# homenc/HElib

Hardware: NVIDIA H100
Metric: ctxt_mults_per_s (higher is better)
Workload: dtype u64

## Files before the change

### helib_b200/csrc/hb_device.cuh

```cuda
#pragma once

#ifdef HB_SIM
#include "cusim.h"
#define HB_SMEM_DECL
#define HB_SMEM ((u64*)cusim::smem_)
#define HB_NOINLINE __attribute__((noinline))
#define HB_GRID_CONSTANT
#else
#define HB_GRID_CONSTANT __grid_constant__
#define HB_NOINLINE __noinline__
#include <cuda_runtime.h>
#define HB_LAUNCH(kernel, grid, block, smem, stream, ...) kernel<<<(grid), (block), (smem), (stream)>>>(__VA_ARGS__)
#define HB_SMEM_DECL extern __shared__ unsigned long long hb_smem_[];
#define HB_SMEM hb_smem_
#endif

#include <stdint.h>

typedef unsigned long long u64;
typedef long long i64;

#define HB_MAXROWS 64
#ifndef HB_MAXB
#define HB_MAXB 64
// ... 262 lines not shown
  const size_t rowoff = (size_t)pi << J.logN;
  const u64* src = J.src[blockIdx.z] + rowoff;
  u64* dst = J.dst[blockIdx.z] + rowoff;
  const unsigned u0 = blockIdx.x << J.logwb;

  for (int e = tid; e < (wb << lb); e += nthr) {
    int v = e >> J.logwb, ub = e & (wb - 1);
    unsigned c = hb_brev(v, lb);
    T[ub * RS + c] = src[((size_t)v << n1) + u0 + ub];
  }
  __syncthreads();
  for (int s = lb - 1; s >= 0; s--) {
    const int logt = lb - 1 - s;
    for (int e = tid; e < (wb << (lb - 1)); e += nthr) {
      int ub = e >> (lb - 1), bf = e & ((BLK >> 1) - 1);
      int i = bf >> logt, o = bf & ((1 << logt) - 1);
      int j = (i << (logt + 1)) + o;
      unsigned b = hb_brev(u0 + ub, n1);
      ulonglong2 tw = P.iw[((size_t)1 << (n1 + s)) + ((size_t)b << s) + i];
      u64* pa = T + ub * RS + j;
      u64* pb = pa + (1 << logt);
      u64 U = *pa, V = *pb;
      *pa = hb_addmod(U, V, q);
      *pb = hb_mul_shoup(hb_submod(U, V, q), tw.x, tw.y, q);
    }
    __syncthreads();
  }
  for (int e = tid; e < (wb << lb); e += nthr) {
    int ub = e >> lb, c = e & (BLK - 1);
    unsigned b = hb_brev(u0 + ub, n1);
    dst[((size_t)b << lb) + c] = T[ub * RS + c];
  }
}

__device__ __forceinline__ void hb_cols_load(u64* T, const u64* src, int n1, int lb, int logw, unsigned c0) {
  const int cnt = 1 << (n1 + logw);
  for (int e = threadIdx.x; e < cnt; e += blockDim.x) {
    int i1 = e >> logw, c = e & ((1 << logw) - 1);
    T[e] = src[((size_t)i1 << lb) + c0 + c];
  }
}
__device__ __forceinline__ void hb_cols_store(const u64* T, u64* dst, int n1, int lb, int logw, unsigned c0) {
  const int cnt = 1 << (n1 + logw);
  for (int e = threadIdx.x; e < cnt; e += blockDim.x) {
    int i1 = e >> logw, c = e & ((1 << logw) - 1);
    dst[((size_t)i1 << lb) + c0 + c] = T[e];
  }
}

__global__ void __launch_bounds__(HB_THREADS) k_fwd_cols(const HbPrimeDev* __restrict__ primes, HbColsJob J) {
  HB_SMEM_DECL
  u64* T = HB_SMEM;
  const int n1 = J.logN - J.log_blk;
  const int pi = J.rows.prime[blockIdx.y];
  const HbPrimeDev P = primes[pi];
  const size_t rowoff = (size_t)pi << J.logN;
  const unsigned c0 = blockIdx.x << J.logw;
  hb_cols_load(T, J.src[blockIdx.z] + rowoff, n1, J.log_blk, J.logw, c0);
  __syncthreads();
  hb_tile_fwd_cols(T, n1, J.logw, P.fw, P.q);
  hb_cols_store(T, J.dst[blockIdx.z] + rowoff, n1, J.log_blk, J.logw, c0);
}

__global__ void __launch_bounds__(HB_THREADS) k_inv_cols(const HbPrimeDev* __restrict__ primes, HbColsJob J) {
  HB_SMEM_DECL
  u64* T = HB_SMEM;
  const int n1 = J.logN - J.log_blk;
  const int pi = J.rows.prime[blockIdx.y];
  const HbPrimeDev P = primes[pi];
  const size_t rowoff = (size_t)pi << J.logN;
  const unsigned c0 = blockIdx.x << J.logw;
  hb_cols_load(T, J.src[blockIdx.z] + rowoff, n1, J.log_blk, J.logw, c0);
  __syncthreads();
  hb_tile_inv_cols(T, n1, J.logw, P.iw, P.q);
  const int cnt = 1 << (n1 + J.logw);
  for (int e = threadIdx.x; e < cnt; e += blockDim.x) T[e] = hb_mul_shoup(T[e], P.ninv, P.ninv_s, P.q);
  __syncthreads();
  hb_cols_store(T, J.dst[blockIdx.z] + rowoff, n1, J.log_blk, J.logw, c0);
}


#define HB_MAXL 66

__device__ HB_NOINLINE int hb_crt_exact(const HbConvDev* cv, const u64* y, int ystride, int* sign, u64* xout, int Lout, int positive) {
  const int n = cv->n, L = cv->L;
  u64 X[HB_MAXL + 1];
  for (int l = 0; l <= L; l++) X[l] = 0;
  for (int j = 0; j < n; j++) {
    const u64 yj = y[(size_t)j * ystride];
    const u64* Qj = cv->Qj + (size_t)j * L;
    u64 carry = 0;
    for (int l = 0; l < L; l++) {
      u64 lo = yj * Qj[l], hi = __umul64hi(yj, Qj[l]);
      u64 s = X[l] + lo; u64 c1 = s < lo;
      u64 s2 = s + carry; u64 c2 = s2 < carry;
      X[l] = s2; carry = hi + c1 + c2;
    }
    X[L] += carry;
  }
  int v = 0;
  for (;;) {
    bool neg = (X[L] >> 63) != 0;
    int cmp = 0;
    if (neg) cmp = -1;
    else if (X[L] != 0) cmp = 1;
    else {
      for (int l = L - 1; l >= 0; l--) {
        u64 bl = positive ? cv->Q[l] : cv->Qhalf[l];
        if (X[l] != bl) { cmp = X[l] < bl ? -1 : 1; break; }
      }
      if (positive && cmp == 0) cmp = 1;
    }
    if (cmp <= 0) break;
    u64 borrow = 0;
    for (int l = 0; l < L; l++) {
      u64 a = X[l], b = cv->Q[l];
      u64 d = a - b; u64 b1 = a < b;
      u64 d2 = d - borrow; u64 b2 = d < borrow;
      X[l] = d2; borrow = b1 + b2;
    }
    X[L] -= borrow;
    v++;
  }
  bool neg = (X[L] >> 63) != 0;
  bool zero = true;
  for (int l = 0; l <= L; l++) if (X[l]) zero = false;
  *sign = neg ? -1 : (zero ? 0 : 1);
  if (xout) {
    u64 ext = neg ? ~0ULL : 0ULL;
    for (int l = 0; l < Lout; l++) xout[l] = l <= L ? X[l] : ext;
  }
  return v;
}

__device__ __forceinline__ i64 hb_conv_v(const HbConvDev* cv, const u64* y, int ystride, u64* stats, double* frac = nullptr, bool bgv = true) {
  const int n = cv->n;
  u64 shi = 0, slo = 0;
  for (int j = 0; j < n; j++) {
    const u64 yj = y[(size_t)j * ystride];
    u64 m = cv->fmul[j];
    int sh = cv->fshift[j];
    u64 lo = yj * m, hi = __umul64hi(yj, m);
    u64 f = sh == 0 ? lo : ((lo >> sh) | (hi << (64 - sh)));
    slo += f;
    shi += (slo < f) ? 1ULL : 0ULL;
  }
  u64 F = slo + 0x8000000000000000ULL;
  i64 v = (i64)(shi + (F < slo ? 1ULL : 0ULL));
  const u64 margin = 4ULL * (u64)n;
  int sign = 2;
  if (F >= 0 - margin) {
    const i64 ve = hb_crt_exact(cv, y, ystride, &sign, nullptr, 0, 0);
    if (ve != v) F = 0;
    v = ve;
    if (stats) atomicAdd(stats, 1ULL);
  }
  if (bgv && cv->has_p) {
    const u64 p = cv->p;
    u64 hi = 0, lo = 0;
    for (int j = 0; j < n; j++) hb_mac128(hi, lo, y[(size_t)j * ystride], cv->cp[j]);
    hb_mac128(hi, lo, (u64)v, cv->negQ_p);
    u64 u = hb_reduce128(hi, lo, p, cv->p_c64, cv->p_c64_s, cv->p_one_s);
    if (u != 0) {
      u = hb_mul_shoup(u, cv->Qinv_p, cv->Qinv_p_s, p);
      const u64 half = p >> 1;
      bool minus = u > half;
      if (!minus && (p & 1ULL) == 0 && u == half) {
        if (sign == 2) {
          if (F >= 0x8000000000000000ULL) sign = 1;
          else if (F < 0x8000000000000000ULL - margin) sign = -1;
          else { hb_crt_exact(cv, y, ystride, &sign, nullptr, 0, 0); if (stats) atomicAdd(stats, 1ULL); }
        }
        minus = sign < 0;
      }
      const i64 v2 = minus ? (i64)u - (i64)p : (i64)u;
      v += v2;
      if (frac) *frac = (double)(i64)(F ^ 0x8000000000000000ULL) * 5.421010862427522e-20 - (double)v2;
      return v;
    }
  }
  if (frac) *frac = (double)(i64)(F ^ 0x8000000000000000ULL) * 5.421010862427522e-20;
  return v;
}

__global__ void __launch_bounds__(HB_THREADS) k_conv(const HbPrimeDev* __restrict__ primes, HbConvJob J) {
  HB_SMEM_DECL
  const HbConvDev* cv = J.cv;
  const int n = cv->n, nt = cv->nt;
  const int n1 = J.logN - J.log_blk, lb = J.log_blk, logw = J.logw;
  const int TILE = 1 << (n1 + logw);
  u64* Y = HB_SMEM;
  i64* Vb = (i64*)(Y + (size_t)n * TILE);
  u64* W = (u64*)(Vb + TILE);
  const int tid = threadIdx.x, nthr = blockDim.x;
  const unsigned c0 = blockIdx.x << logw;
  const u64* src = J.src[blockIdx.y];
  u64* dst = J.dst[blockIdx.y];

  for (int j = 0; j < n; j++) {
    const int pi = cv->src_prime[j];
    const HbPrimeDev P = primes[pi];
    u64* T = Y + (size_t)j * TILE;
    hb_cols_load(T, src + ((size_t)pi << J.logN), n1, lb, logw, c0);
    __syncthreads();
    if (J.src_is_y) continue;
    hb_tile_inv_cols(T, n1, logw, P.iw, P.q);
    const u64 t = cv->tn[j], ts = cv->tn_s[j];
    for (int e = tid; e < TILE; e += nthr) T[e] = hb_mul_shoup(T[e], t, ts, P.q);
  }
  __syncthreads();
  double* fr = J.frac[blockIdx.y];
  for (int e = tid; e < TILE; e += nthr) {
    double f;
    Vb[e] = hb_conv_v(cv, Y + e, TILE, J.stats, fr ? &f : nullptr);
    if (fr) fr[((size_t)(e >> logw) << lb) + c0 + (e & ((1 << logw) - 1))] = f;
  }
  __syncthreads();
  for (int t = 0; t < nt; t++) {
    const int pi = cv->tgt_prime[t];
    const HbPrimeDev P = primes[pi];
    const u64* ct = cv->c + (size_t)t * n;
    const u64 nq = cv->negQ[t], pq = cv->Qmod[t];
    for (int e = tid; e < TILE; e += nthr) {
      u64 hi = 0, lo = 0;
      for (int j = 0; j < n; j++) hb_mac128(hi, lo, Y[(size_t)j * TILE + e], ct[j]);
      i64 v = Vb[e];
      if (v >= 0) hb_mac128(hi, lo, (u64)v, nq);
      else hb_mac128(hi, lo, (u64)(-v), pq);
      W[e] = hb_reduce128(hi, lo, P);
    }
    __syncthreads();
    hb_tile_fwd_cols(W, n1, logw, P.fw, P.q);
    hb_cols_store(W, dst + ((size_t)pi << J.logN), n1, lb, logw, c0);
    __syncthreads();
  }
}

struct HbCrtTabs { const u64* t; const u64* t_s; };
__global__ void __launch_bounds__(HB_THREADS) k_crt(const HbPrimeDev* __restrict__ primes, HbCrtJob J, HbCrtTabs tabs) {
  const HbConvDev* cv = J.cv;
  const int n = cv->n;
  size_t k = (size_t)blockIdx.x * blockDim.x + threadIdx.x;
  if (k >= (size_t)J.N) return;
  u64 y[HB_MAXROWS];
  for (int j = 0; j < n; j++) {
    int pi = cv->src_prime[j];
    u64 q = primes[pi].q;
    y[j] = hb_mul_shoup(J.src[(size_t)pi * J.N + k], tabs.t[j], tabs.t_s[j], q);
  }
  int sign;
  hb_crt_exact(cv, y, 1, &sign, J.out + k * J.Lout, J.Lout, J.positive);
}

__global__ void __launch_bounds__(HB_THREADS) k_crt_modp(const HbPrimeDev* __restrict__ primes, HbCrtJob J, HbCrtTabs tabs) {
// ... 548 lines not shown
```

### helib_b200/csrc/hb_device_v1.cuh

```cuda
#pragma once
#include <utility>
#include "hb_device.cuh"

#define HB1_RS 17
#define HB1_BS 273

__device__ __forceinline__ void hb_group_sync(int group, int nthreads) {
#ifdef HB_SIM
  cusim::bar_sync(1 + group, nthreads);
#else
  asm volatile("bar.sync %0, %1;" ::"r"(1 + group), "r"(nthreads) : "memory");
#endif
}

__device__ __forceinline__ void hb1_mac128(u64& hi, u64& lo, u64 a, u64 b) {
#ifdef HB_SIM
  hb_mac128(hi, lo, a, b);
#else
  asm("{\n\t.reg .u64 pl, ph;\n\t"
      "mul.lo.u64 pl, %2, %3;\n\t"
      "mul.hi.u64 ph, %2, %3;\n\t"
      "add.cc.u64 %0, %0, pl;\n\t"
      "addc.u64 %1, %1, ph;\n\t}"
      : "+l"(lo), "+l"(hi)
// ... 495 lines not shown
  u64* peer[8][HB_MAXB];
};

template <bool SP>
__global__ void __launch_bounds__(256, 2) k1_fwd_cols(const HbPrimeDev* __restrict__ primes, const HB_GRID_CONSTANT Hb1ColsJob J) {
  HB_SMEM_DECL
  u64* T = HB_SMEM;
  const int tid = threadIdx.x;
  const int pi = J.rows.prime[blockIdx.y];
  const HbPrimeDev P = primes[pi];
  HB1_MOD(M, P);
  const size_t rowoff = (size_t)pi << J.logN;
  const unsigned c0 = blockIdx.x << 4;
  const int c = tid & 15, x = tid >> 4;
  Hb1TwPtr tw1;
  tw1.p[0] = P.fw + 1; tw1.p[1] = P.fw + 2; tw1.p[2] = P.fw + 4; tw1.p[3] = P.fw + 8;
  Hb1TwReg tw2;
  tw2.load([&](int k, int g) { return P.fw[(16 << k) + (x << k) + g]; });
  for (int it = blockIdx.z; it < J.nitems; it += gridDim.z) {
    const u64* src = J.src[it] + rowoff + c0 + c;
    u64* dst = J.dst[it] + rowoff + c0 + c;
    u64 a[16];
    hb1_unroll<16>([&](auto r) { a[r] = src[(size_t)(16 * r + x) << 8]; });
    hb1_r16_fwd<SP>(a, tw1, M);
    hb1_unroll<16>([&](auto r) { T[c * HB1_BS + HB1_RS * r + x] = a[r]; });
    __syncthreads();
    hb1_unroll<16>([&](auto l) { a[l] = T[c * HB1_BS + HB1_RS * x + l]; });
    hb1_r16_fwd<SP>(a, tw2, M);
    hb1_unroll<16>([&](auto l) { dst[(size_t)(16 * x + l) << 8] = a[l]; });
    __syncthreads();
  }
}
template <bool SP>
__global__ void __launch_bounds__(256, 2) k1_inv_cols(const HbPrimeDev* __restrict__ primes, const HB_GRID_CONSTANT Hb1ColsJob J) {
  HB_SMEM_DECL
  u64* T = HB_SMEM;
  const int tid = threadIdx.x;
  const int pi = J.rows.prime[blockIdx.y];
  const HbPrimeDev P = primes[pi];
  const u64 q = P.q; HB1_MOD(M, P);
  const size_t rowoff = (size_t)pi << J.logN;
  const unsigned c0 = blockIdx.x << 4;
  const int c = tid & 15, x = tid >> 4;
  Hb1TwPtr tw1;
  tw1.p[0] = P.iw + 1; tw1.p[1] = P.iw + 2; tw1.p[2] = P.iw + 4; tw1.p[3] = P.iw + 8;
  Hb1TwReg tw2;
  tw2.load([&](int k, int g) { return P.iw[(16 << k) + (x << k) + g]; });
  for (int it = blockIdx.z; it < J.nitems; it += gridDim.z) {
    const u64* src = J.src[it] + rowoff + c0 + c;
    u64* dst = J.dst[it] + rowoff + c0 + c;
    u64 a[16];
    hb1_unroll<16>([&](auto l) { a[l] = src[(size_t)(16 * x + l) << 8]; });
    hb1_r16_inv<SP>(a, tw2, M);
    hb1_unroll<16>([&](auto l) { T[c * HB1_BS + HB1_RS * x + l] = a[l]; });
    __syncthreads();
    hb1_unroll<16>([&](auto r) { a[r] = T[c * HB1_BS + HB1_RS * r + x]; });
    hb1_r16_inv<SP>(a, tw1, M);
    const u64 fm = J.has_scal ? J.scal[blockIdx.y] : P.ninv, fs = J.has_scal ? J.scal_s[blockIdx.y] : P.ninv_s;
    hb1_unroll<16>([&](auto r) {
      const u64 v = hb_mul_shoup(a[r], fm, fs, q);
      const size_t o = (size_t)(16 * r + x) << 8;
      dst[o] = v;
      for (int p = 0; p < J.npeers; p++) J.peer[p][it][rowoff + c0 + c + o] = v;
    });
    __syncthreads();
  }
}

#define HB1C_BS 276
#define HB1_TS (4 * HB1C_BS)
#define HB1_VS 260

struct Hb1ConvJob {
  const HbConvDev* cv;
  int logN, ngroups;
  int nitems;
  const u64* src[HB_MAXB];
  u64* dst[HB_MAXB];
  u64* stats;
  int src_is_y;
  double* frac[HB_MAXB];
};

template <bool SP>
__global__ void __launch_bounds__(640, 1) k1_conv(const HbPrimeDev* __restrict__ primes, const HB_GRID_CONSTANT Hb1ConvJob J) {
  HB_SMEM_DECL
  const HbConvDev* cv = J.cv;
  const int n = cv->n, nt = cv->nt, NG = J.ngroups;
  u64* Y = HB_SMEM;
  i64* Vb = (i64*)(Y + (size_t)n * HB1_TS);
  u64* W = (u64*)(Vb + 4 * HB1_VS);
  const int tid = threadIdx.x;
  const int grp = tid >> 6, gt = tid & 63;
  const int c = gt & 3, x = gt >> 2;
  const unsigned c0 = blockIdx.x << 2;
  const u64* src = J.src[blockIdx.y];
  u64* dst = J.dst[blockIdx.y];

  for (int j = grp; j < n; j += NG) {
    const int pi = cv->src_prime[j];
    const HbPrimeDev P = primes[pi];
    const u64 q = P.q; HB1_MOD(M, P);
    const u64* s = src + ((size_t)pi << J.logN) + c0 + c;
    u64* Yj = Y + (size_t)j * HB1_TS + c * HB1C_BS;
    u64 a[16];
    hb1_unroll<16>([&](auto l) { a[l] = s[(size_t)(16 * x + l) << 8]; });
    if (J.src_is_y) {
      hb1_unroll<16>([&](auto l) { Yj[HB1_RS * x + l] = a[l]; });
      continue;
    }
    {
      Hb1TwPtr tw;
      tw.p[0] = P.iw + 16 + x; tw.p[1] = P.iw + 32 + 2 * x; tw.p[2] = P.iw + 64 + 4 * x; tw.p[3] = P.iw + 128 + 8 * x;
      hb1_r16_inv<SP>(a, tw, M);
    }
    hb1_unroll<16>([&](auto l) { Yj[HB1_RS * x + l] = a[l]; });
    hb_group_sync(grp, 64);
    hb1_unroll<16>([&](auto r) { a[r] = Yj[HB1_RS * r + x]; });
    {
      Hb1TwPtr tw;
      tw.p[0] = P.iw + 1; tw.p[1] = P.iw + 2; tw.p[2] = P.iw + 4; tw.p[3] = P.iw + 8;
      hb1_r16_inv<SP>(a, tw, M);
    }
    const u64 t = cv->tn[j], ts = cv->tn_s[j];
    hb1_unroll<16>([&](auto r) { Yj[HB1_RS * r + x] = hb_mul_shoup(a[r], t, ts, q); });
  }
  __syncthreads();
  for (int e = tid; e < 1024; e += blockDim.x) {
    const int cc = e >> 8, i1 = e & 255;
    double* fr = J.frac[blockIdx.y];
    double f;
    Vb[cc * HB1_VS + i1] = hb_conv_v(cv, Y + cc * HB1C_BS + HB1_RS * (i1 >> 4) + (i1 & 15), HB1_TS, J.stats, fr ? &f : nullptr);
    if (fr) fr[((size_t)i1 << 8) + c0 + cc] = f;
  }
  __syncthreads();
  u64* Wg = W + (size_t)grp * HB1_TS + c * HB1C_BS;
  for (int t = grp; t < nt; t += NG) {
    const int pi = cv->tgt_prime[t];
    const HbPrimeDev P = primes[pi];
    HB1_MOD(M, P);
    const u64* ct = cv->c + (size_t)t * n;
    u64 a[16];
    {
      const u64 negq = cv->negQ[t], posq = cv->Qmod[t];
      hb1_unroll<2>([&](auto h) {
        u64 ahi[8], alo[8];
        hb1_unroll<8>([&](auto r) {
          const i64 v = Vb[c * HB1_VS + 16 * (8 * h + r) + x];
          const u64 m = v >= 0 ? (u64)v : (u64)(-v);
          const u64 f = v >= 0 ? negq : posq;
          if ((m >> 32) == 0) {
            const u64 p0 = hb1_mulwide((unsigned)m, (unsigned)f);
            const u64 p1 = hb1_mulwide((unsigned)m, (unsigned)(f >> 32)) + (p0 >> 32);
            alo[r] = (p1 << 32) | (unsigned)p0; ahi[r] = p1 >> 32;
          } else { alo[r] = m * f; ahi[r] = __umul64hi(m, f); }
        });
        for (int j = 0; j < n; j++) {
          const u64 cj = ct[j];
          const u64* Yj = Y + (size_t)j * HB1_TS + c * HB1C_BS + x + HB1_RS * 8 * h;
          hb1_unroll<8>([&](auto r) { hb1_mac128(ahi[r], alo[r], Yj[HB1_RS * r], cj); });
        }
        hb1_unroll<8>([&](auto r) { a[8 * h + r] = hb_reduce128_lazy(ahi[r], alo[r], P); });
      });
    }
    {
      Hb1TwPtr tw;
      tw.p[0] = P.fw + 1; tw.p[1] = P.fw + 2; tw.p[2] = P.fw + 4; tw.p[3] = P.fw + 8;
      hb1_r16_fwd<SP>(a, tw, M);
    }
    hb_group_sync(grp, 64);
    hb1_unroll<16>([&](auto r) { Wg[HB1_RS * r + x] = a[r]; });
    hb_group_sync(grp, 64);
    hb1_unroll<16>([&](auto l) { a[l] = Wg[HB1_RS * x + l]; });
    {
      Hb1TwPtr tw;
      tw.p[0] = P.fw + 16 + x; tw.p[1] = P.fw + 32 + 2 * x; tw.p[2] = P.fw + 64 + 4 * x; tw.p[3] = P.fw + 128 + 8 * x;
      hb1_r16_fwd<SP>(a, tw, M);
    }
    u64* d = dst + ((size_t)pi << J.logN) + c0 + c;
    hb1_unroll<16>([&](auto l) { d[(size_t)(16 * x + l) << 8] = a[l]; });
  }
}

struct Hb1Conv1Job {
  int logN, ngroups, cq, nitems;
  int src_prime, nt;
  int tgt_prime[HB_MAXROWS];
  u64 qs_mod[HB_MAXROWS];
  unsigned char nored[HB_MAXROWS];
  u64 ninv, ninv_s;
  const u64* src[HB_MAXB];
  u64* dst[HB_MAXB];
};
template <bool SP>
__global__ void __launch_bounds__(640, 1) k1_conv1(const HbPrimeDev* __restrict__ primes, const HB_GRID_CONSTANT Hb1Conv1Job J) {
  HB_SMEM_DECL
  const int NG = J.ngroups, CQ = J.cq, nt = J.nt;
  u64* Y = HB_SMEM;
  u64* W = Y + (size_t)CQ * HB1_TS;
  const int tid = threadIdx.x;
  const int grp = tid >> 6, gt = tid & 63;
  const int c = gt & 3, x = gt >> 2;
  const unsigned c0 = blockIdx.x * 4u * (unsigned)CQ;
  const u64* src = J.src[blockIdx.y];
  u64* dst = J.dst[blockIdx.y];
  const HbPrimeDev PS = primes[J.src_prime];
  for (int qd = grp; qd < CQ; qd += NG) {
    HB1_MOD(M, PS);
    const u64* s = src + ((size_t)J.src_prime << J.logN) + c0 + 4 * qd + c;
    u64* Yq = Y + (size_t)qd * HB1_TS + c * HB1C_BS;
    u64 a[16];
    hb1_unroll<16>([&](auto l) { a[l] = s[(size_t)(16 * x + l) << 8]; });
    {
      Hb1TwPtr tw;
      tw.p[0] = PS.iw + 16 + x; tw.p[1] = PS.iw + 32 + 2 * x; tw.p[2] = PS.iw + 64 + 4 * x; tw.p[3] = PS.iw + 128 + 8 * x;
      hb1_r16_inv<SP>(a, tw, M);
    }
    hb1_unroll<16>([&](auto l) { Yq[HB1_RS * x + l] = a[l]; });
    hb_group_sync(grp, 64);
    hb1_unroll<16>([&](auto r) { a[r] = Yq[HB1_RS * r + x]; });
    {
      Hb1TwPtr tw;
      tw.p[0] = PS.iw + 1; tw.p[1] = PS.iw + 2; tw.p[2] = PS.iw + 4; tw.p[3] = PS.iw + 8;
      hb1_r16_inv<SP>(a, tw, M);
    }
    hb1_unroll<16>([&](auto r) { Yq[HB1_RS * r + x] = hb_mul_shoup(a[r], J.ninv, J.ninv_s, PS.q); });
  }
  __syncthreads();
  const u64 qs_half = (PS.q - 1) >> 1;
  u64* Wg = W + (size_t)grp * HB1_TS + c * HB1C_BS;
  for (int w = grp; w < nt * CQ; w += NG) {
    const int t = w / CQ, qd = w - t * CQ;
    const int pi = J.tgt_prime[t];
    const HbPrimeDev P = primes[pi];
    HB1_MOD(M, P);
    const u64 adj = P.q - J.qs_mod[t];
    const u64* Yq = Y + (size_t)qd * HB1_TS + c * HB1C_BS + x;
    const bool nored = J.nored[t] != 0;
    u64 a[16];
    hb1_unroll<16>([&](auto r) {
      const u64 y = Yq[HB1_RS * r];
      u64 v = nored ? y : y - __umul64hi(y, P.one_s) * P.q;
      if (y > qs_half) v += adj;
      a[r] = v;
    });
    {
      Hb1TwPtr tw;
      tw.p[0] = P.fw + 1; tw.p[1] = P.fw + 2; tw.p[2] = P.fw + 4; tw.p[3] = P.fw + 8;
      hb1_r16_fwd<SP>(a, tw, M);
    }
    hb_group_sync(grp, 64);
    hb1_unroll<16>([&](auto r) { Wg[HB1_RS * r + x] = a[r]; });
    hb_group_sync(grp, 64);
    hb1_unroll<16>([&](auto l) { a[l] = Wg[HB1_RS * x + l]; });
    {
      Hb1TwPtr tw;
      tw.p[0] = P.fw + 16 + x; tw.p[1] = P.fw + 32 + 2 * x; tw.p[2] = P.fw + 64 + 4 * x; tw.p[3] = P.fw + 128 + 8 * x;
      hb1_r16_fwd<SP>(a, tw, M);
    }
    u64* d = dst + ((size_t)pi << J.logN) + c0 + 4 * qd + c;
    hb1_unroll<16>([&](auto l) { d[(size_t)(16 * x + l) << 8] = a[l]; });
  }
}

// ... 161 lines not shown
```

### helib_b200/csrc/hb_engine.cu

```cuda
#include "hb_device.cuh"
#include "hb_device_v1.cuh"
#include "hb_device_v2.cuh"
#include "hb_device_gen.cuh"
#include "hb_device_prg.cuh"

#include <algorithm>
#include <cmath>
#include <cstdarg>
#include <cstdio>
#include <cstdlib>
#include <cstring>
#include <map>
#include <set>
#include <string>
#include <vector>

#include "../../include/helib_b200.h"

typedef unsigned __int128 u128;

static size_t blk_parts_smem(int nparts) {
  return (2 * HB1_STAGE + 16 * 256 + (nparts - 1) * 16 * 256) * sizeof(u64) + 256 * sizeof(ulonglong2);
}

// ... 1064 lines not shown
    if (p >= (1ULL << 62)) return hb_fail(HB_ERR_UNSUPPORTED, "ptxt_space >= 2^62");
    u64 Qp = prod_mod_excl(-1, p), Qinv;
    if (!h_invmod(Qp, p, &Qinv)) return hb_fail(HB_ERR_BAD_ARG, "ptxt_space %llu is not coprime to the dropped primes", (unsigned long long)p);
    H.p = p; H.p_c64 = (u64)(((u128)1 << 64) % p); H.p_c64_s = h_shoup(H.p_c64, p); H.p_one_s = (u64)(((u128)1 << 64) / p);
    H.Qinv_p = Qinv; H.Qinv_p_s = h_shoup(Qinv, p);
    H.negQ_p = Qp ? p - Qp : 0;
    for (int j = 0; j < n; j++) cp[j] = prod_mod_excl(j, p);
  }
  std::vector<unsigned char> blob;
  auto put = [&](const void* src_, size_t bytes) { size_t off = (blob.size() + 15) & ~(size_t)15; blob.resize(off + bytes); memcpy(&blob[off], src_, bytes); return off; };
  size_t o_src = put(h_src.data(), sizeof(int) * n), o_tgt = put(h_tgt.data(), sizeof(int) * std::max(nt, 1));
  size_t o_fs = put(fshift.data(), sizeof(int) * n);
  size_t o_t = put(t.data(), 8 * n), o_ts = put(t_s.data(), 8 * n), o_tn = put(tn.data(), 8 * n), o_tns = put(tn_s.data(), 8 * n);
  size_t o_fm = put(fmul.data(), 8 * n), o_c = put(cmat.data(), 8 * std::max<size_t>(cmat.size(), 1));
  size_t o_nq = put(negQ.data(), 8 * std::max(nt, 1)), o_qm = put(Qmod.data(), 8 * std::max(nt, 1)), o_cp = put(cp.data(), 8 * n);
  size_t o_Q = put(Q.data(), 8 * L), o_Qh = put(Qhalf.data(), 8 * L), o_Qj = put(Qj.data(), 8 * (size_t)n * L);
  HB_TRY(ctx_alloc(c, &E.blob, blob.size()));
  HB_CUDA(cudaMemcpy(E.blob, blob.data(), blob.size(), cudaMemcpyHostToDevice));
  unsigned char* B = (unsigned char*)E.blob;
  H.src_prime = (const int*)(B + o_src); H.tgt_prime = (const int*)(B + o_tgt); H.fshift = (const int*)(B + o_fs);
  E.d_t = (const u64*)(B + o_t); E.d_t_s = (const u64*)(B + o_ts);
  H.tn = (const u64*)(B + o_tn); H.tn_s = (const u64*)(B + o_tns); H.fmul = (const u64*)(B + o_fm);
  H.c = (const u64*)(B + o_c); H.negQ = (const u64*)(B + o_nq); H.Qmod = (const u64*)(B + o_qm); H.cp = (const u64*)(B + o_cp);
  H.Q = (const u64*)(B + o_Q); H.Qhalf = (const u64*)(B + o_Qh); H.Qj = (const u64*)(B + o_Qj);
  HB_TRY(ctx_alloc(c, (void**)&E.d, sizeof(HbConvDev)));
  HB_CUDA(cudaMemcpy(E.d, &H, sizeof(HbConvDev), cudaMemcpyHostToDevice));
  auto ins = c->convs.emplace(key, E);
  *out = &ins.first->second;
  return HB_OK;
}

static int norm_scratch(hb_ctx* c) {
  if (c->d_frac) return HB_OK;
  HB_TRY(ctx_alloc(c, (void**)&c->d_frac, (size_t)HB_MAXB * c->N * sizeof(double)));
  HB_TRY(ctx_alloc(c, (void**)&c->d_z, (size_t)HB_MAXB * c->N * 2 * sizeof(double)));
  HB_TRY(ctx_alloc(c, (void**)&c->d_max, HB_MAXB * sizeof(unsigned long long)));
  return HB_OK;
}
static int norm_chunk(hb_ctx* c, int nit, double* out) {
  HbNormJob J; J.logN = c->logN; J.npoly = nit; J.frac = c->d_frac; J.z = (double2*)c->d_z; J.maxbits = c->d_max;
  HB_CUDA(cudaMemsetAsync(c->d_max, 0, nit * sizeof(unsigned long long), c->stream));
  unsigned gx = (unsigned)std::max<size_t>(1, c->N / (HB_THREADS * 4));
  pre_launch(c);
  HB_LAUNCH(k_norm_twist, dim3(gx, nit), dim3(HB_THREADS), 0, c->stream, J);
  HB_TRY(post_launch(c, "k_norm_twist", (u64)nit * c->N * 24));
  for (int logd = c->logN - 1; logd >= 0; logd--) {
    pre_launch(c);
    HB_LAUNCH(k_norm_stage, dim3(gx, nit), dim3(HB_THREADS), 0, c->stream, J, logd, logd == 0 ? 1 : 0);
    HB_TRY(post_launch(c, "k_norm_stage", (u64)nit * c->N * 32));
  }
  unsigned long long bits[HB_MAXB];
  HB_CUDA(cudaMemcpyAsync(bits, c->d_max, nit * sizeof(unsigned long long), cudaMemcpyDeviceToHost, c->stream));
  HB_CUDA(cudaStreamSynchronize(c->stream));
  for (int i = 0; i < nit; i++) { double m2; memcpy(&m2, &bits[i], 8); out[i] = std::sqrt(m2); }
  return HB_OK;
}
static int conv_chunk(hb_ctx* c, u64* const* polys, int nit, const int32_t* src, int n, const int32_t* tgt, int nt, u64 p, int src_is_y = 0, bool want_frac = false) {
  HB_TRY(ctx_scratch(c));
  if (want_frac) HB_TRY(norm_scratch(c));
  ConvEntry* E; HB_TRY(get_conv(c, src, n, tgt, nt, p, &E));
  u64* tA[HB_MAXB]; u64* tB[HB_MAXB];
  tmp_ptrs(c, c->tmpA, nit, tA); tmp_ptrs(c, c->tmpB, nit, tB);
  if (src_is_y) { for (int i = 0; i < nit; i++) tA[i] = polys[i]; }
  else HB_TRY(launch_blk(c, -1, (const u64* const*)polys, tA, nit, src, n, 0, nullptr));
  if (v1_cols_ok(c) && c->conv1 && n == 1 && p <= 1 && !src_is_y && !want_frac && nt <= HB_MAXROWS) {
    Hb1Conv1Job J1; memset(&J1, 0, sizeof(J1));
    static const int cq_env = [] { const char* e = getenv("HB_CONV1_CQ"); int v = e ? atoi(e) : 0; return (v == 1 || v == 2 || v == 4) ? v : 0; }();
    const int cq = cq_env ? cq_env : 4, ng = 10;
    J1.logN = c->logN; J1.ngroups = ng; J1.cq = cq; J1.nitems = nit; J1.src_prime = src[0]; J1.nt = nt;
    const u64 qs = c->q[src[0]];
    for (int t = 0; t < nt; t++) { J1.tgt_prime[t] = tgt[t]; J1.qs_mod[t] = qs % c->q[tgt[t]]; J1.nored[t] = (u128)qs <= (u128)7 * c->q[tgt[t]] ? 1 : 0; }
    u64 ninv; if (!h_invmod(c->N % qs, qs, &ninv)) return hb_fail(HB_ERR_BAD_ARG, "N not invertible");
    J1.ninv = ninv; J1.ninv_s = h_shoup(ninv, qs);
    for (int i = 0; i < nit; i++) { J1.src[i] = tA[i]; J1.dst[i] = tB[i]; }
    const size_t smem1 = (size_t)(cq + ng) * HB1_TS * sizeof(u64);
    pre_launch(c);
    if (all_special(c)) HB_LAUNCH(k1_conv1<true>, dim3(64 / cq, nit), dim3(64 * ng), smem1, c->stream, c->d_primes, J1);
    else HB_LAUNCH(k1_conv1<false>, dim3(64 / cq, nit), dim3(64 * ng), smem1, c->stream, c->d_primes, J1);
    return post_launch(c, "k1_conv1", (u64)(n + nt) * nit * c->N * 8);
  }
  if (v1_cols_ok(c)) {
    int ng = 0; double best = -1; size_t smem1 = 0;
    for (int g = 10; g >= 4; g--) {
      size_t sm = ((size_t)(n + g) * HB1_TS + 4 * HB1_VS) * sizeof(u64);
      if (sm > 224 * 1024) continue;
      int by_smem = (int)((227 * 1024) / (sm + 1024)), by_regs = 65536 / (96 * 64 * g);
      int ctas = std::max(1, std::min(std::min(by_smem, by_regs), 2));
      double work = n + 1.4 * nt, slots = (double)((n + g - 1) / g) + 1.4 * ((nt + g - 1) / g);
      double balance = work / (slots * g);
      double warps = std::min(20.0, 2.0 * g * ctas);
      double score = balance * (0.5 + 0.5 * warps / 20.0) * (ctas >= 2 ? 1.15 : 1.0);
      if (score > best) { best = score; ng = g; smem1 = sm; }
    }
    if (ng > 0) {
      Hb1ConvJob J1; memset(&J1, 0, sizeof(J1));
      J1.cv = E->d; J1.logN = c->logN; J1.ngroups = ng; J1.nitems = nit; J1.stats = c->d_stats; J1.src_is_y = src_is_y;
      if (want_frac) for (int i = 0; i < nit; i++) J1.frac[i] = c->d_frac + (size_t)i * c->N;
      for (int i = 0; i < nit; i++) { J1.src[i] = tA[i]; J1.dst[i] = tB[i]; }
      pre_launch(c);
      if (all_special(c)) HB_LAUNCH(k1_conv<true>, dim3(64, nit), dim3(64 * ng), smem1, c->stream, c->d_primes, J1);
      else HB_LAUNCH(k1_conv<false>, dim3(64, nit), dim3(64 * ng), smem1, c->stream, c->d_primes, J1);
      return post_launch(c, "k1_conv", (u64)(n + nt) * nit * c->N * 8);
    }
  }
  const int n1 = c->logN - c->log_blk;
  int lw = logw_cols(c);
  while (lw > 0 && ((size_t)(n + 2) << (n1 + lw)) * sizeof(u64) > c->max_smem) lw--;
  size_t smem = ((size_t)(n + 2) << (n1 + lw)) * sizeof(u64);
  if (smem > c->max_smem) return hb_fail(HB_ERR_UNSUPPORTED, "base conversion tile needs %zu bytes of shared memory", smem);
  HbConvJob J; memset(&J, 0, sizeof(J));
  J.cv = E->d; J.logN = c->logN; J.log_blk = c->log_blk; J.logw = lw; J.nitems = nit; J.stats = c->d_stats; J.src_is_y = src_is_y;
  if (want_frac) for (int i = 0; i < nit; i++) J.frac[i] = c->d_frac + (size_t)i * c->N;
  for (int i = 0; i < nit; i++) { J.src[i] = tA[i]; J.dst[i] = tB[i]; }
  dim3 grid(1u << (c->log_blk - lw), nit);
  pre_launch(c);
  HB_LAUNCH(k_conv, grid, dim3(HB_THREADS), smem, c->stream, c->d_primes, J);
  return post_launch(c, "k_conv", (u64)(n + nt) * nit * c->N * 8);
}

struct PlanScope {
  hb_ctx* c; int logN, log_blk; HbPrimeDev* dp; size_t N;
  PlanScope(hb_ctx* c_, int plan) : c(c_), logN(c_->logN), log_blk(c_->log_blk), dp(c_->d_primes), N(c_->N) {
    if (plan == 0) { c->logN = c->gen.logL; c->log_blk = c->gen.log_blk_L; c->d_primes = c->gen.d_primes_cyc; c->N = c->gen.L; }
    else { c->logN = c->gen.logL2; c->log_blk = c->gen.log_blk_L2; c->d_primes = c->gen.d_primes_cyc2; c->N = c->gen.L2; }
  }
  ~PlanScope() { c->logN = logN; c->log_blk = log_blk; c->d_primes = dp; c->N = N; }
};
static long h_phi(long m) { long r = m, n = m; for (long p = 2; p * p <= n; p++) if (n % p == 0) { while (n % p == 0) n /= p; r -= r / p; } if (n > 1) r -= r / n; return r; }
static long h_gcd(long a, long b) { while (b) { long t = a % b; a = b; b = t; } return a; }
static bool h_isprime_small(long n) { if (n < 2) return false; for (long p = 2; p * p <= n; p++) if (n % p == 0) return false; return true; }
static u64 h_find_primitive_root(u64 q, u64 e) {
  u64 root = 1, n = e;
  for (u64 p = 2; p <= n; p++) {
    if (n % p) continue;
    u64 pp = 1; while (n % p == 0) { n /= p; pp *= p; }
    u64 g = 2;
    for (;; g++) if (h_isprime_small((long)g) && h_powmod(g, (q - 1) / p, q) != 1) break;
    root = h_mulmod(root, h_powmod(g, (q - 1) / pp, q), q);
  }
  return root;
}
static void poly_mul_binom(std::vector<long>& a, long k) { std::vector<long> r(a.size() + k, 0); for (size_t i = 0; i < a.size(); i++) { r[i + k] += a[i]; r[i] -= a[i]; } a.swap(r); }
static void poly_div_binom(std::vector<long>& a, long k) {
  std::vector<long> qv(a.size() - k, 0);
  for (long i = (long)a.size() - 1; i >= k; i--) { long cq = a[i]; qv[i - k] = cq; a[i] -= cq; a[i - k] += cq; }
  a.swap(qv);
}
static int h_mobius(long n) { int mu = 1; for (long p = 2; p * p <= n; p++) if (n % p == 0) { n /= p; if (n % p == 0) return 0; mu = -mu; } if (n > 1) mu = -mu; return mu; }
static std::vector<long> h_cyclotomic(long m) {
  std::vector<long> a(1, 1);
  for (long d = 1; d <= m; d++) if (m % d == 0 && h_mobius(d) == 1) poly_mul_binom(a, m / d);
  for (long d = 1; d <= m; d++) if (m % d == 0 && h_mobius(d) == -1) poly_div_binom(a, m / d);
  return a;
}

static int gen_cyc_ntt(hb_ctx* c, int dir, u64* const* w, u64* const* tmp, int nit, const int32_t* idx, int n, int plan = 0) {
  PlanScope ps(c, plan);
  if (dir > 0) { HB_TRY(launch_cols(c, +1, (const u64* const*)w, tmp, nit, idx, n)); return launch_blk(c, +1, (const u64* const*)tmp, w, nit, idx, n, 0, nullptr); }
  HB_TRY(launch_blk(c, -1, (const u64* const*)w, tmp, nit, idx, n, 0, nullptr));
  return launch_cols(c, -1, (const u64* const*)tmp, w, nit, idx, n);
}
static int gen_k(hb_ctx* c, int op, int which, const u64* const* src, u64* const* dst, int nit, const int32_t* idx, int n) {
  hb_ctx::Gen& g = c->gen;
  for (int r0 = 0; r0 < n; r0 += HB_MAXROWS) {
    int nr = std::min(HB_MAXROWS, n - r0);
    HbGenJob J; memset(&J, 0, sizeof(J));
    J.m = g.m; J.phim = g.phim; J.L = g.L; J.L2 = g.L2; J.d = g.d; J.rep = g.d_rep; J.irep = g.d_irep; J.which = which;
// ... 2028 lines not shown
```

Baseline: 3047.

## Defer exact CRT fallback out of conv loop and stage coefficients in shared memory

The fast-base-conversion kernel now defers rare exact-CRT fallback elements into a shared-memory worklist. A second pass resolves them with an inlined exact CRT whose multiword scratch lives in shared memory, replacing the noinline call with a local-memory array. This is meant to remove call and local-memory overhead and register pressure from the main V loop. The conversion matrix and the negQ/Qmod constants are also copied into shared memory so the MAC loop reads them there rather than from global memory, which grows the shared-memory footprint and can change the group-count choice. Optional clock64 phase stamps and a microbenchmark script are added for profiling.

```diff
diff --git a/bench_micro/conv_phases.py b/bench_micro/conv_phases.py
--- /dev/null
+++ b/bench_micro/conv_phases.py
@@ -0,0 +1,82 @@
+import argparse
+import collections
+import os
+import re
+import subprocess
+import sys
+import tempfile
+
+ROOT = os.path.dirname(os.path.dirname(os.path.abspath(__file__)))
+sys.path.insert(0, ROOT)
+SRC = os.path.join(ROOT, "bench_micro", "ubench_conv.cu")
+FLAGS = ["-gencode", "arch=compute_90a,code=sm_90a", "-O3", "-std=c++17"]
+
+
+def shapes():
+    from helib_b200 import Chain
+    ch = Chain(1 << 17, -1, 1, 1190, 2)
+    S = ch.ctxt[:-1]
+    out = []
+    for d in ch.digits:
+        rows = sorted(set(d) & set(S))
+        if rows:
+            out.append((rows, sorted(set(S + ch.special) - set(rows)), 32))
+    out.append((ch.special, S, 64))
+    return ch, out
+
+
+def sass_report(nvcc, tmp):
+    cubin = os.path.join(tmp, "conv.cubin")
+    r = subprocess.run([nvcc] + FLAGS + ["-cubin", "-Xptxas", "-v", SRC, "-o", cubin], check=True, capture_output=True, text=True)
+    cur = None
+    for ln in (r.stdout + r.stderr).splitlines():
+        m = re.search(r"Function properties for (_Z7k1_conv\w+)", ln)
+        if m:
+            cur = m.group(1)
+        elif cur and ("stack frame" in ln or "registers" in ln):
+            print(cur, ln.strip())
+            if "registers" in ln:
+                cur = None
+    objdump = os.path.join(os.path.dirname(nvcc), "cuobjdump")
+    sass = subprocess.run([objdump, "-sass", "-fun", "_Z7k1_convILb1EEvPK10HbPrimeDev10Hb1ConvJob", cubin],
+                          check=True, capture_output=True, text=True).stdout
+    ins = []
+    for ln in sass.splitlines():
+        m = re.match(r"\s*/\*([0-9a-f]{4,})\*/\s+(@!?U?P\w+\s+)?([A-Z][A-Z0-9_.]*)\s*([^;]*);", ln)
+        if m:
+            ins.append((int(m.group(1), 16), m.group(3), m.group(4)))
+    mix = lambda seq: collections.Counter(op.split(".")[0] + (".WIDE" if ".WIDE" in op else "") + (".HI" if ".HI" in op else "")
+                                          for _, op, _ in seq)
+    print("k1_conv<true>: %d instructions, mix %s" % (len(ins), dict(mix(ins).most_common(14))))
+    for addr, op, arg in ins:
+        m = re.search(r"0x([0-9a-f]+)", arg) if op == "BRA" else None
+        if m and int(m.group(1), 16) < addr:
+            body = [t for t in ins if int(m.group(1), 16) <= t[0] <= addr]
+            w = sum(1 for t in body if "IMAD.WIDE" in t[1])
+            local = sum(1 for t in body if t[1].startswith(("LDL", "STL")))
+            if w >= 64 and len(body) < 600:
+                print("MAC loop 0x%s-0x%x: %d instructions per iteration, %d local-memory, mix %s"
+                      % (m.group(1), addr, len(body), local, dict(mix(body).most_common(10))))
+
+
+def main():
+    ap = argparse.ArgumentParser(description=__doc__, formatter_class=argparse.RawDescriptionHelpFormatter)
+    ap.add_argument("--sass", action="store_true", help="report ptxas -v and the SASS instruction mix (no GPU)")
+    args = ap.parse_args()
+    from helib_b200.build import _nvcc
+    nvcc = _nvcc()
+    with tempfile.TemporaryDirectory() as tmp:
+        if args.sass:
+            return sass_report(nvcc, tmp)
+        ch, shp = shapes()
+        argv = [str(ch.m), ",".join(str(q) for q in ch.primes)]
+        argv += ["%s:%s:%d" % (",".join(map(str, s)), ",".join(map(str, t)), it) for s, t, it in shp]
+        for name, extra in (("plain", []), ("stamps", ["-DHB_CONV_STAMPS"])):
+            exe = os.path.join(tmp, "ubench_conv_" + name)
+            subprocess.run([nvcc] + FLAGS + extra + [SRC, "-o", exe], check=True)
+            print("# " + name, flush=True)
+            subprocess.run([exe] + argv, check=True)
+
+
+if __name__ == "__main__":
+    main()
diff --git a/bench_micro/ubench_conv.cu b/bench_micro/ubench_conv.cu
--- /dev/null
+++ b/bench_micro/ubench_conv.cu
@@ -0,0 +1,112 @@
+#include "../helib_b200/csrc/hb_engine.cu"
+
+#include <algorithm>
+#include <sstream>
+
+#define CK(x) do { int r_ = (x); if (r_ != HB_OK) { fprintf(stderr, "%s:%d %s\n", __FILE__, __LINE__, hb_last_error()); return 1; } } while (0)
+#define CKC(x) do { cudaError_t e_ = (x); if (e_ != cudaSuccess) { fprintf(stderr, "%s:%d %s\n", __FILE__, __LINE__, cudaGetErrorString(e_)); return 1; } } while (0)
+
+__global__ void k_fill(u64* rows, const u64* q, int np, size_t N, u64 seed) {
+  const size_t n = (size_t)np * N;
+  for (size_t i = (size_t)blockIdx.x * blockDim.x + threadIdx.x; i < n; i += (size_t)gridDim.x * blockDim.x) {
+    u64 z = seed + i * 0x9E3779B97F4A7C15ULL;
+    z = (z ^ (z >> 30)) * 0xBF58476D1CE4E5B9ULL; z = (z ^ (z >> 27)) * 0x94D049BB133111EBULL; z ^= z >> 31;
+    rows[i] = z % q[i / N];
+  }
+}
+
+static std::vector<long long> parse_list(const std::string& s) {
+  std::vector<long long> v; std::stringstream ss(s); std::string t;
+  while (std::getline(ss, t, ',')) if (!t.empty()) v.push_back(std::stoll(t));
+  return v;
+}
+
+static double kernel_ms(hb_ctx* c, const char* want) {
+  char name[64]; uint64_t launches = 0; double ms = 0;
+  for (int i = 0; hb_ctx_profile_get(c, i, name, sizeof(name), &launches, &ms, nullptr) == HB_OK; i++)
+    if (!strcmp(name, want)) return ms / (double)launches;
+  return -1;
+}
+
+int main(int argc, char** argv) {
+  if (argc < 4) { fprintf(stderr, "usage: %s m q0,q1,... src:tgt:items ...\n", argv[0]); return 2; }
+  const u64 m = std::stoull(argv[1]);
+  std::vector<u64> q; for (long long v : parse_list(argv[2])) q.push_back((u64)v);
+  const int np = (int)q.size();
+  hb_ctx* c; CK(hb_ctx_create(&c, 0, m, np, (const uint64_t*)q.data(), nullptr));
+  const size_t N = c->N;
+  u64* dq; CKC(cudaMalloc(&dq, np * sizeof(u64)));
+  CKC(cudaMemcpy(dq, q.data(), np * sizeof(u64), cudaMemcpyHostToDevice));
+  for (int a = 3; a < argc; a++) {
+    std::string sh = argv[a];
+    const size_t p1 = sh.find(':'), p2 = sh.find(':', p1 + 1);
+    std::vector<int32_t> src, tgt;
+    for (long long v : parse_list(sh.substr(0, p1))) src.push_back((int32_t)v);
+    for (long long v : parse_list(sh.substr(p1 + 1, p2 - p1 - 1))) tgt.push_back((int32_t)v);
+    const int nit = std::stoi(sh.substr(p2 + 1)), n = (int)src.size(), nt = (int)tgt.size();
+    u64* buf; CKC(cudaMalloc(&buf, (size_t)nit * np * N * sizeof(u64)));
+    k_fill<<<1024, 256>>>(buf, dq, np, N, 0x5eed0000ULL + a);
+    CKC(cudaDeviceSynchronize());
+    std::vector<u64*> polys(nit);
+    for (int i = 0; i < nit; i++) polys[i] = buf + (size_t)i * np * N;
+#ifdef HB_CONV_STAMPS
+    const size_t cells = (size_t)nit * 64 * 10 * 8;
+    u64* dst_; CKC(cudaMalloc(&dst_, cells * sizeof(u64)));
+    CKC(cudaMemcpyToSymbol(hb1c_stamps, &dst_, sizeof(dst_)));
+#endif
+    for (int w = 0; w < 3; w++) CK(conv_chunk(c, polys.data(), nit, src.data(), n, tgt.data(), nt, 1));
+    CK(hb_ctx_reset_stats(c));
+    std::vector<double> rounds;
+    for (int r = 0; r < 5; r++) {
+      CK(hb_ctx_profile(c, 1));
+      for (int k = 0; k < 20; k++) CK(conv_chunk(c, polys.data(), nit, src.data(), n, tgt.data(), nt, 1));
+      CK(hb_ctx_profile(c, 0));
+      rounds.push_back(kernel_ms(c, "k1_conv"));
+    }
+    std::sort(rounds.begin(), rounds.end());
+    uint64_t st[3]; CK(hb_ctx_stats(c, st));
+    std::vector<u64> h((size_t)nt * N);
+    u64 hash = 1469598103934665603ULL;
+    for (int i = 0; i < nit; i++) {
+      for (int t = 0; t < nt; t++)
+        CKC(cudaMemcpy(h.data() + (size_t)t * N, c->tmpB + ((size_t)i * np + tgt[t]) * N, N * sizeof(u64), cudaMemcpyDeviceToHost));
+      for (u64 v : h) { hash ^= v; hash *= 1099511628211ULL; }
+    }
+    printf("{\"shape\": [%d, %d, %d], \"k1_conv_ms\": {\"best\": %.4f, \"median\": %.4f}, \"exact_fallbacks\": %llu, \"hash\": \"%016llx\"",
+           n, nt, nit, rounds[0], rounds[2], (unsigned long long)st[0], (unsigned long long)hash);
+#ifdef HB_CONV_STAMPS
+    CKC(cudaMemset(dst_, 0, cells * sizeof(u64)));
+    CK(conv_chunk(c, polys.data(), nit, src.data(), n, tgt.data(), nt, 1));
+    CKC(cudaDeviceSynchronize());
+    std::vector<u64> s(cells);
+    CKC(cudaMemcpy(s.data(), dst_, cells * sizeof(u64), cudaMemcpyDeviceToHost));
+    double acc[8] = {0}, cta = 0; long groups = 0, ctas = 0; int ng = 0;
+    for (size_t b = 0; b < (size_t)nit * 64; b++) {
+      const u64* g = &s[b * 80];
+      u64 t0 = ~0ULL, t7 = 0; int k = 0;
+      for (; k < 10 && g[8 * k]; k++) { t0 = std::min(t0, g[8 * k]); t7 = std::max(t7, g[8 * k + 7]); }
+      ng = k;
+      for (int j = 0; j < k; j++) {
+        const u64* e = g + 8 * j;
+        acc[0] += e[1] - e[0]; acc[1] += e[2] - e[1]; acc[2] += e[3] - e[2]; acc[3] += e[4] - e[3];
+        acc[4] += e[5]; acc[5] += e[6]; acc[6] += t7 - e[7];
+        acc[7] += (e[7] - e[4]) - e[5] - e[6];
+        groups++;
+      }
+      cta += t7 - t0; ctas++;
+    }
+    const char* names[8] = {"src", "bar1", "v", "bar2", "mac", "xf", "idle", "other"};
+    cta /= ctas;
+    printf(", \"groups\": %d, \"cta_cycles\": %.0f, \"phases\": {", ng, cta);
+    for (int k = 0; k < 8; k++) printf("%s\"%s\": [%.0f, %.3f]", k ? ", " : "", names[k], acc[k] / groups, acc[k] / groups / cta);
+    printf("}");
+    cudaFree(dst_);
+#endif
+    printf("}\n");
+    fflush(stdout);
+    cudaFree(buf);
+  }
+  cudaFree(dq);
+  hb_ctx_destroy(c);
+  return 0;
+}
diff --git a/helib_b200/csrc/hb_device.cuh b/helib_b200/csrc/hb_device.cuh
--- a/helib_b200/csrc/hb_device.cuh
+++ b/helib_b200/csrc/hb_device.cuh
@@ -368,9 +368,8 @@
 
 #define HB_MAXL 66
 
-__device__ HB_NOINLINE int hb_crt_exact(const HbConvDev* cv, const u64* y, int ystride, int* sign, u64* xout, int Lout, int positive) {
+__device__ __forceinline__ int hb_crt_exact_x(const HbConvDev* cv, const u64* y, int ystride, int* sign, u64* xout, int Lout, int positive, u64* X) {
   const int n = cv->n, L = cv->L;
-  u64 X[HB_MAXL + 1];
   for (int l = 0; l <= L; l++) X[l] = 0;
   for (int j = 0; j < n; j++) {
     const u64 yj = y[(size_t)j * ystride];
@@ -418,8 +417,19 @@
   }
   return v;
 }
-
-__device__ __forceinline__ i64 hb_conv_v(const HbConvDev* cv, const u64* y, int ystride, u64* stats, double* frac = nullptr, bool bgv = true) {
+__device__ HB_NOINLINE int hb_crt_exact(const HbConvDev* cv, const u64* y, int ystride, int* sign, u64* xout, int Lout, int positive) {
+  u64 X[HB_MAXL + 1];
+  return hb_crt_exact_x(cv, y, ystride, sign, xout, Lout, positive, X);
+}
+
+enum { HB_EXACT_CALL, HB_EXACT_DEFER, HB_EXACT_INLINE };
+template <int EXACT = HB_EXACT_CALL>
+__device__ __forceinline__ i64 hb_conv_v(const HbConvDev* cv, const u64* y, int ystride, u64* stats, double* frac = nullptr, bool bgv = true,
+                                         bool* deferred = nullptr, u64* X = nullptr) {
+  auto crt_exact = [&](int* sg) {
+    if constexpr (EXACT == HB_EXACT_INLINE) return hb_crt_exact_x(cv, y, ystride, sg, nullptr, 0, 0, X);
+    else return hb_crt_exact(cv, y, ystride, sg, nullptr, 0, 0);
+  };
   const int n = cv->n;
   u64 shi = 0, slo = 0;
   for (int j = 0; j < n; j++) {
@@ -436,7 +446,8 @@
   const u64 margin = 4ULL * (u64)n;
   int sign = 2;
   if (F >= 0 - margin) {
-    const i64 ve = hb_crt_exact(cv, y, ystride, &sign, nullptr, 0, 0);
+    if (EXACT == HB_EXACT_DEFER) { *deferred = true; return 0; }
+    const i64 ve = crt_exact(&sign);
     if (ve != v) F = 0;
     v = ve;
     if (stats) atomicAdd(stats, 1ULL);
@@ -455,7 +466,8 @@
         if (sign == 2) {
           if (F >= 0x8000000000000000ULL) sign = 1;
           else if (F < 0x8000000000000000ULL - margin) sign = -1;
-          else { hb_crt_exact(cv, y, ystride, &sign, nullptr, 0, 0); if (stats) atomicAdd(stats, 1ULL); }
+          else if (EXACT == HB_EXACT_DEFER) { *deferred = true; return 0; }
+          else { crt_exact(&sign); if (stats) atomicAdd(stats, 1ULL); }
         }
         minus = sign < 0;
       }
diff --git a/helib_b200/csrc/hb_device_v1.cuh b/helib_b200/csrc/hb_device_v1.cuh
--- a/helib_b200/csrc/hb_device_v1.cuh
+++ b/helib_b200/csrc/hb_device_v1.cuh
@@ -601,6 +601,20 @@
   double* frac[HB_MAXB];
 };
 
+#ifdef HB_CONV_STAMPS
+__device__ unsigned long long* hb1c_stamps;
+#define HB1C_STAMP_INIT u64* st_ = hb1c_stamps + ((size_t)(blockIdx.y * gridDim.x + blockIdx.x) * 10 + grp) * 8; \
+  u64 st_mac = 0, st_xf = 0, st_t0 = 0, st_t1 = 0
+#define HB1C_STAMP(k) do { if (gt == 0) st_[k] = clock64(); } while (0)
+#define HB1C_MARK(v) (v) = clock64()
+#define HB1C_STAMP_END do { if (gt == 0) { st_[5] = st_mac; st_[6] = st_xf; st_[7] = clock64(); } } while (0)
+#else
+#define HB1C_STAMP_INIT
+#define HB1C_STAMP(k)
+#define HB1C_MARK(v)
+#define HB1C_STAMP_END
+#endif
+
 template <bool SP>
 __global__ void __launch_bounds__(640, 1) k1_conv(const HbPrimeDev* __restrict__ primes, const HB_GRID_CONSTANT Hb1ConvJob J) {
   HB_SMEM_DECL
@@ -608,13 +622,21 @@
   const int n = cv->n, nt = cv->nt, NG = J.ngroups;
   u64* Y = HB_SMEM;
   i64* Vb = (i64*)(Y + (size_t)n * HB1_TS);
-  u64* W = (u64*)(Vb + 4 * HB1_VS);
+  u64* Cs = (u64*)(Vb + 4 * HB1_VS);
+  u64* nslow = Cs + (size_t)nt * (n + 2);
+  u64* W = nslow + 1;
   const int tid = threadIdx.x;
   const int grp = tid >> 6, gt = tid & 63;
   const int c = gt & 3, x = gt >> 2;
   const unsigned c0 = blockIdx.x << 2;
   const u64* src = J.src[blockIdx.y];
   u64* dst = J.dst[blockIdx.y];
+  HB1C_STAMP_INIT;
+  HB1C_STAMP(0);
+  int* slow = (int*)W;
+  if (tid == 0) *nslow = 0;
+  for (int i = tid; i < nt * n; i += blockDim.x) Cs[i] = cv->c[i];
+  for (int t = tid; t < nt; t += blockDim.x) { Cs[nt * n + t] = cv->negQ[t]; Cs[nt * (n + 1) + t] = cv->Qmod[t]; }
 
   for (int j = grp; j < n; j += NG) {
     const int pi = cv->src_prime[j];
@@ -644,24 +666,43 @@
     const u64 t = cv->tn[j], ts = cv->tn_s[j];
     hb1_unroll<16>([&](auto r) { Yj[HB1_RS * r + x] = hb_mul_shoup(a[r], t, ts, q); });
   }
+  HB1C_STAMP(1);
   __syncthreads();
+  HB1C_STAMP(2);
+  double* fr = J.frac[blockIdx.y];
   for (int e = tid; e < 1024; e += blockDim.x) {
     const int cc = e >> 8, i1 = e & 255;
-    double* fr = J.frac[blockIdx.y];
     double f;
-    Vb[cc * HB1_VS + i1] = hb_conv_v(cv, Y + cc * HB1C_BS + HB1_RS * (i1 >> 4) + (i1 & 15), HB1_TS, J.stats, fr ? &f : nullptr);
+    bool deferred = false;
+    const i64 v = hb_conv_v<HB_EXACT_DEFER>(cv, Y + cc * HB1C_BS + HB1_RS * (i1 >> 4) + (i1 & 15), HB1_TS, J.stats, &f, true, &deferred);
+    if (deferred) { slow[atomicAdd(nslow, 1ULL)] = e; continue; }
+    Vb[cc * HB1_VS + i1] = v;
     if (fr) fr[((size_t)i1 << 8) + c0 + cc] = f;
   }
+  HB1C_STAMP(3);
   __syncthreads();
+  if (const int ns = (int)*nslow) {
+    const int room = (NG * HB1_TS - 512) / (cv->L + 1), nx = room < (int)blockDim.x ? room : (int)blockDim.x;
+    for (int k = tid; tid < nx && k < ns; k += nx) {
+      const int e = slow[k], cc = e >> 8, i1 = e & 255;
+      double f;
+      Vb[cc * HB1_VS + i1] = hb_conv_v<HB_EXACT_INLINE>(cv, Y + cc * HB1C_BS + HB1_RS * (i1 >> 4) + (i1 & 15), HB1_TS, J.stats, &f, true,
+                                                        nullptr, W + 512 + (size_t)tid * (cv->L + 1));
+      if (fr) fr[((size_t)i1 << 8) + c0 + cc] = f;
+    }
+    __syncthreads();
+  }
+  HB1C_STAMP(4);
   u64* Wg = W + (size_t)grp * HB1_TS + c * HB1C_BS;
   for (int t = grp; t < nt; t += NG) {
     const int pi = cv->tgt_prime[t];
     const HbPrimeDev P = primes[pi];
     HB1_MOD(M, P);
-    const u64* ct = cv->c + (size_t)t * n;
+    const u64* ct = Cs + (size_t)t * n;
     u64 a[16];
+    HB1C_MARK(st_t0);
     {
-      const u64 negq = cv->negQ[t], posq = cv->Qmod[t];
+      const u64 negq = Cs[nt * n + t], posq = Cs[nt * (n + 1) + t];
       hb1_unroll<2>([&](auto h) {
         u64 ahi[8], alo[8];
         hb1_unroll<8>([&](auto r) {
@@ -682,6 +723,7 @@
         hb1_unroll<8>([&](auto r) { a[8 * h + r] = hb_reduce128_lazy(ahi[r], alo[r], P); });
       });
     }
+    HB1C_MARK(st_t1);
     {
       Hb1TwPtr tw;
       tw.p[0] = P.fw + 1; tw.p[1] = P.fw + 2; tw.p[2] = P.fw + 4; tw.p[3] = P.fw + 8;
@@ -698,7 +740,11 @@
     }
     u64* d = dst + ((size_t)pi << J.logN) + c0 + c;
     hb1_unroll<16>([&](auto l) { d[(size_t)(16 * x + l) << 8] = a[l]; });
-  }
+#ifdef HB_CONV_STAMPS
+    st_mac += st_t1 - st_t0; st_xf += clock64() - st_t1;
+#endif
+  }
+  HB1C_STAMP_END;
 }
 
 struct Hb1Conv1Job {
diff --git a/helib_b200/csrc/hb_engine.cu b/helib_b200/csrc/hb_engine.cu
--- a/helib_b200/csrc/hb_engine.cu
+++ b/helib_b200/csrc/hb_engine.cu
@@ -1170,7 +1170,7 @@
   if (v1_cols_ok(c)) {
     int ng = 0; double best = -1; size_t smem1 = 0;
     for (int g = 10; g >= 4; g--) {
-      size_t sm = ((size_t)(n + g) * HB1_TS + 4 * HB1_VS) * sizeof(u64);
+      size_t sm = ((size_t)(n + g) * HB1_TS + 4 * HB1_VS + (size_t)nt * (n + 2) + 1) * sizeof(u64);
       if (sm > 224 * 1024) continue;
       int by_smem = (int)((227 * 1024) / (sm + 1024)), by_regs = 65536 / (96 * 64 * g);
       int ctas = std::max(1, std::min(std::min(by_smem, by_regs), 2));
```

After: 3062 (median of 6 runs). No clear change (+0.5%).
